# swapna267/flink

Measured on AMD Instinct MI355X. Metric: windowed-agg events/sec (whole node) at 1/2/4/8 GPU + % of HBM peak, higher is better.
Workload: dtype int64; 1 GPU; cfg2: Nexmark Q7-style TUMBLE(10 s) MAX(price) GROUP BY auction; plan=one-phase, keys_total=1000000, superbuckets=1024

## Files before the change

### flink_amd/csrc/fw_merge_impl.h

```cpp
#pragma once
#include <type_traits>

#include "fw_kernel_common.h"

namespace fw {
template <int NW, int E>
struct StateLds {
    static constexpr int NI = mg_idx_slots(NW, E);
    uint32_t idx[NI];
    int64_t key[E];
    int64_t slice[E];
    uint32_t flag[E];
    uint64_t acc[NW][E];
    uint16_t due[E];
    int32_t ndue;
    int32_t n;
    uint32_t overflow;
};

constexpr uint32_t IDX_DEAD = 0xFFFFFFFFu;

template <int W>
__device__ __forceinline__ void load_words(const uint64_t* p, uint64_t (&o)[W]) {
    if constexpr (W % 2 == 0) {
// ... 678 lines not shown
};
__device__ __forceinline__ CellGroup cell_group(uint32_t v, int f, int64_t CH) {
    const int lane = threadIdx.x & 63;
    const uint32_t cnt = cell_count(v);
    uint32_t inc = cnt;
#pragma unroll
    for (int d = 1; d < 64; d <<= 1) {
        const uint32_t t = (uint32_t)__shfl_up((int)inc, d, 64);
        if (lane >= d) inc += t;
    }
    CellGroup g;
    g.tot = (uint32_t)__shfl((int)inc, 63, 64);
    g.excl = inc - cnt;
    g.adj = (uint32_t)(cell_chunk(f) * CH + cell_start(v)) - g.excl;
    g.fmt = cell_fmt(v);
    return g;
}
constexpr int GF_PASS = 1;
constexpr int GF_COMPACT = 2;

struct PackDec {
    int64_t kbase, vbase, rbase;
    uint32_t ksh, rb, vb;
};
__device__ __forceinline__ PackDec pack_dec(const MergeArgs& a) {
    PackDec d;
    const uint32_t bits = __hip_atomic_load(&a.ctrl->pk_cur_bits, __ATOMIC_RELAXED, DEV_SCOPE);
    d.kbase = __hip_atomic_load(&a.ctrl->pk_cur_k, __ATOMIC_RELAXED, DEV_SCOPE);
    d.vbase = __hip_atomic_load(&a.ctrl->pk_cur_v, __ATOMIC_RELAXED, DEV_SCOPE);
    d.rbase = a.slot_base[0];
    d.ksh = 64u - (bits & 255u);
    d.rb = (bits >> 8) & 255u;
    d.vb = (bits >> 16) & 255u;
    return d;
}
template <int PW>
__device__ __forceinline__ void unpack_row(const PackDec& d, uint64_t w, int64_t interval, uint64_t (&row)[PW]) {
    static_assert(PW == 3, "PF_PACK rows carry one accumulator word");
    row[0] = (uint64_t)d.kbase + (w >> d.ksh);
    const uint32_t rank = (uint32_t)(w >> d.vb) & ((1u << d.rb) - 1u);
    row[1] = (uint64_t)(d.rbase + (int64_t)(rank * (uint32_t)interval));
    row[2] = (uint64_t)d.vbase + (w & ((1ull << d.vb) - 1ull));
}

template <int NW, int GU, int GF>
__device__ __forceinline__ uint32_t load_group_rows(const MergeArgs& a, int64_t pi, const CellGroup& g, uint32_t r0,
                                                    int sb, uint64_t (&row)[GU][2 + NW]) {
    constexpr int PW = 2 + NW;
    constexpr bool PS = (GF & GF_PASS) != 0, CR = (GF & GF_COMPACT) != 0;
    const int lane = threadIdx.x & 63;
    const uint64_t* seg = a.parts + (size_t)pi * a.cap_rows * PW;
#pragma unroll
    for (int u = 0; u < GU; u++) {
        const uint32_t x = min(r0 + (uint32_t)(u * 64 + lane), g.tot - 1);
        int lo = 0;
#pragma unroll
        for (int step = 32; step > 0; step >>= 1)
            if ((uint32_t)__shfl((int)g.excl, lo + step, 64) <= x) lo += step;
        const uint32_t rg = (uint32_t)__shfl((int)g.adj, lo, 64) + x;
        const uint32_t fmt = (uint32_t)__shfl((int)g.fmt, lo, 64);
        if (!CR || fmt == PF_WIDE) {
            load_words<PW>(seg + (size_t)rg * PW, row[u]);
        } else if (NW == 1 && fmt == PF_PACK) {
            const uint32_t within = rg & ((1u << a.ch_log2) - 1u);
            if constexpr (NW == 1) unpack_row(pack_dec(a), seg[(size_t)(rg - within) * PW + within], a.win.interval, row[u]);
        } else {
            const uint32_t within = rg & ((1u << a.ch_log2) - 1u);
            const uint64_t* p = seg + (size_t)(rg - within) * PW;
            const uint32_t rank = a.ranks[(size_t)pi * a.cap_rows + rg];
            row[u][1] = (uint64_t)(a.slot_base[pi] + (int64_t)(rank * (uint32_t)a.win.interval));
            if (fmt == PF_NARROW) {
                uint64_t t[1 + NW];
                load_words<1 + NW>(p + (size_t)within * (1 + NW), t);
                row[u][0] = t[0];
#pragma unroll
                for (int w = 0; w < NW; w++) row[u][2 + w] = t[1 + w];
            } else {
                row[u][0] = p[within];
#pragma unroll
                for (int w = 0; w < NW; w++) row[u][2 + w] = w == 0 ? 1ull : 0ull;
            }
        }
    }
    uint32_t live = 0;
#pragma unroll
    for (int u = 0; u < GU; u++) live |= (uint32_t)(r0 + (uint32_t)(u * 64 + lane) < g.tot) << u;
    if constexpr (PS)
#pragma unroll
        for (int u = 0; u < GU; u++) {
            uint32_t m;
            if ((live >> u) & 1u) live &= ~((uint32_t)(route_key(a.ks, (int64_t)row[u][0], 0, &m) != sb) << u);
        }
    return live;
}

static __device__ __noinline__ bool tz_fired_out_of_line(TzTable z, int64_t we, int64_t progress) {
    return tz_is_fired(z, we, progress);
}

static_assert(FW_MAX_PENDING * RUN_X <= 64, "one lane per (push, sub-run)");
struct RunSegs {
    uint32_t tot;
    uint32_t excl;
    uint32_t adj;
    uint32_t pf;
};
__device__ __forceinline__ RunSegs run_segs(const MergeArgs& a, int isb, int64_t pend) {
    const int lane = threadIdx.x & 63;
    const int p = lane / RUN_X, x = lane % RUN_X;
    uint32_t n = 0, fm = 0;
    if (p < pend) {
        n = min(a.run_fill[((size_t)p * RUN_X + x) * a.n_sb + isb], (uint32_t)a.sub_cap);
        fm = (uint32_t)a.slot_fmt[p];
    }
    uint32_t inc = n;
#pragma unroll
    for (int d = 1; d < 64; d <<= 1) {
        const uint32_t t = (uint32_t)__shfl_up((int)inc, d, 64);
        if (lane >= d) inc += t;
    }
    RunSegs g;
    g.tot = (uint32_t)__shfl((int)inc, 63, 64);
    g.excl = inc - n;
    g.adj = (uint32_t)(((size_t)isb * RUN_X + x) * (size_t)a.sub_cap) - g.excl;
    g.pf = (uint32_t)p | (fm << 4);
    return g;
}
template <int GU>
__device__ __forceinline__ uint32_t locate_run_rows(const RunSegs& g, uint32_t r0_, uint32_t (&ri)[GU], uint32_t (&pf)[GU]) {
    const int lane = threadIdx.x & 63;
    const uint32_t r0 = (uint32_t)__builtin_amdgcn_readfirstlane((int)r0_);
    const uint32_t tot = (uint32_t)__builtin_amdgcn_readfirstlane((int)g.tot);
    const uint32_t last = min(r0 + (uint32_t)(64 * GU), tot) - 1u;
    const uint32_t first = min(r0, tot - 1u);
    int cur = 0;
#pragma unroll
    for (int step = 32; step > 0; step >>= 1)
        if ((uint32_t)__builtin_amdgcn_readlane((int)g.excl, cur + step) <= first) cur += step;
    uint32_t x[GU], adj[GU];
    {
        const uint32_t a0 = (uint32_t)__builtin_amdgcn_readlane((int)g.adj, cur);
        const uint32_t p0 = (uint32_t)__builtin_amdgcn_readlane((int)g.pf, cur);
#pragma unroll
        for (int u = 0; u < GU; u++) {
            x[u] = min(r0 + (uint32_t)(u * 64 + lane), tot - 1u);
            adj[u] = a0;
            pf[u] = p0;
        }
    }
    while (cur < 63) {
        const uint32_t b = (uint32_t)__builtin_amdgcn_readlane((int)g.excl, cur + 1);
        if (b > last) break;
        cur++;
        const uint32_t an = (uint32_t)__builtin_amdgcn_readlane((int)g.adj, cur);
        const uint32_t pn = (uint32_t)__builtin_amdgcn_readlane((int)g.pf, cur);
#pragma unroll
        for (int u = 0; u < GU; u++) {
            adj[u] = x[u] >= b ? an : adj[u];
            pf[u] = x[u] >= b ? pn : pf[u];
        }
    }
    uint32_t live = 0;
#pragma unroll
    for (int u = 0; u < GU; u++) {
        ri[u] = adj[u] + x[u];
        live |= (uint32_t)(r0 + (uint32_t)(u * 64 + lane) < tot) << u;
    }
    return live;
}
template <int NW, int GU, int GF>
__device__ __forceinline__ uint32_t load_run_rows(const MergeArgs& a, const RunSegs& g, uint32_t r0_,
                                                  uint64_t (&row)[GU][2 + NW]) {
    constexpr int PW = 2 + NW;
    constexpr bool CR = (GF & GF_COMPACT) != 0;
    PackDec pk{};
    if constexpr (CR && NW == 1) pk = pack_dec(a);
    uint32_t rix[GU], pf[GU];
    const uint32_t live = locate_run_rows<GU>(g, r0_, rix, pf);
#pragma unroll
    for (int u = 0; u < GU; u++) {
        const uint32_t ri = rix[u];
        const uint32_t p = pf[u] & 15u, fmt = (pf[u] >> 4) & 3u;
        const uint64_t* base = a.runs + (size_t)p * a.run_rows * PW;
        if (!CR || fmt == PF_WIDE) {
            const uint64_t* q = base + (size_t)ri * PW;
#pragma unroll
            for (int w = 0; w < PW; w++) row[u][w] = q[w];
        } else if (NW == 1 && fmt == PF_PACK) {
            if constexpr (NW == 1) unpack_row(pk, base[ri], a.win.interval, row[u]);
        } else {
            const uint32_t rank = a.run_ranks[(size_t)p * a.run_rows + ri];
            row[u][1] = (uint64_t)(a.slot_base[p] + (int64_t)(rank * (uint32_t)a.win.interval));
            if (fmt == PF_NARROW) {
                uint64_t t[1 + NW];
                load_words<1 + NW>(base + (size_t)ri * (1 + NW), t);
                row[u][0] = t[0];
#pragma unroll
                for (int w = 0; w < NW; w++) row[u][2 + w] = t[1 + w];
            } else {
                row[u][0] = base[ri];
#pragma unroll
                for (int w = 0; w < NW; w++) row[u][2 + w] = w == 0 ? 1ull : 0ull;
            }
        }
    }
    return live;
}
template <int NW, int G, int GF, int D, typename F>
__device__ __forceinline__ void gather_runs(const MergeArgs& a, int sb, int64_t pend, F&& process) {
    constexpr int PW = 2 + NW;
    constexpr uint32_t STEP = (uint32_t)MG_BLOCK * G;
    const RunSegs g = run_segs(a, sb, pend);
    uint32_t r0 = (uint32_t)(threadIdx.x >> 6) * 64u * G;
    if (r0 >= g.tot) return;
    if constexpr (D > 1) {
        uint64_t buf[D][G][PW];
        uint32_t live[D];
        static_for<D - 1>([&](auto K) {
            constexpr int k = decltype(K)::value;
            live[k] = load_run_rows<NW, G, GF>(a, g, r0 + (uint32_t)k * STEP, buf[k]);
        });
        bool done = false;
        while (!done) {
            static_for<D>([&](auto K) {
                constexpr int k = decltype(K)::value;
                constexpr int kn = (k + D - 1) % D;
                if (done) return;
                live[kn] = load_run_rows<NW, G, GF>(a, g, r0 + (uint32_t)(D - 1) * STEP, buf[kn]);
                process(buf[k], live[k]);
                r0 += STEP;
                done = r0 >= g.tot;
            });
        }
    } else {
        for (; r0 < g.tot; r0 += STEP) {
            uint64_t row[G][PW];
            const uint32_t live = load_run_rows<NW, G, GF>(a, g, r0, row);
            process(row, live);
        }
    }
}
__device__ __forceinline__ uint32_t run_overflow(const MergeArgs& a, int sb, int64_t pend) {
    const int lane = threadIdx.x & 63;
    const bool o = lane < pend && a.run_ovf[(size_t)lane * a.n_sb + sb] != 0;
    return (uint32_t)__ballot(o);
}
__device__ __forceinline__ void run_release(const MergeArgs& a, int sb, int64_t pend) {
    const int t = threadIdx.x;
    if (t >= 64) return;
    const int p = t / RUN_X, x = t % RUN_X;
    if (p >= pend) return;
    a.run_fill[((size_t)p * RUN_X + x) * a.n_sb + sb] = 0u;
    if (x == 0) a.run_ovf[(size_t)p * a.n_sb + sb] = 0u;
}
template <int NW, int GU, int GF, typename F>
__device__ __forceinline__ void gather_cells_push(const MergeArgs& a, int sb, int64_t pi, F&& process) {
    constexpr int PW = 2 + NW;
    constexpr bool PS = (GF & GF_PASS) != 0;
    const int lane = threadIdx.x & 63, wv = threadIdx.x >> 6;
    const int ncell = (int)cell_pad(a.slot_nch[pi]);
    const int G = min(64, ncell / (MG_BLOCK / 64));
    const int ngroups = ncell / G;
    const int pl = PS ? a.ks.pass_log2 : 0;
    const int nis = a.n_sb >> pl;
    const uint32_t* cl = a.cells + (size_t)pi * nis * a.max_nch;
    for (int gi = wv; gi < ngroups; gi += MG_BLOCK / 64) {
        const int f = gi * G + lane;
        const uint32_t v = (lane >= G || cell_chunk(f) >= a.slot_nch[pi]) ? 0u : cl[((size_t)(f >> 4) * nis + (sb >> pl)) * CELL_LANES + (f & 15)];
        const CellGroup cg = cell_group(v, f, a.chunk_rows);
        for (uint32_t r0 = 0; r0 < cg.tot; r0 += 64 * GU) {
            uint64_t row[GU][PW];
            const uint32_t live = load_group_rows<NW, GU, GF>(a, pi, cg, r0, sb, row);
            process(row, live);
        }
    }
}

constexpr int GF_TAG = 4;
constexpr int MG_TAG_LOG2 = 13;
static_assert((1 << MG_TAG_LOG2) == MG_TAG_SLOTS, "tag_slot's shift");
constexpr uint32_t TG_DUE = 1u << 31;
#ifndef FW_TAG_G
#define FW_TAG_G 4
#endif
#ifndef FW_TAG_D
#define FW_TAG_D 1
#endif
struct TagLds {
    uint32_t tag[MG_TAG_SLOTS];
    uint64_t acc[MG_TAG_SLOTS];
    int64_t rk_end[MG_TAG_RANKS];
    uint32_t rk_flag[MG_TAG_RANKS];
    uint16_t due[MG_TAG_SLOTS];
    uint16_t live[MG_TAG_SLOTS];
    uint32_t ndue, nlive;
    uint32_t nfresh;
    uint32_t overflow;
};
struct TagEpoch {
    uint32_t bits;
    bool ok;
    int64_t kbase, vbase, rbase;
};
template <int NW, int E, bool TAG>
struct MergeLds {
    StateLds<NW, E> S;
};
template <int NW, int E>
struct MergeLds<NW, E, true> {
    union {
        StateLds<NW, E> S;
        TagLds T;
    };
};
__device__ __forceinline__ uint32_t tag_slot(uint32_t tg) { return (tg * 0x9E3779B1u) >> (32 - MG_TAG_LOG2); }

__device__ __forceinline__ TagEpoch tag_epoch(const MergeArgs& a, int64_t pend, bool flush) {
    TagEpoch ep;
    ep.bits = __hip_atomic_load(&a.ctrl->pk_cur_bits, __ATOMIC_RELAXED, DEV_SCOPE);
    ep.kbase = __hip_atomic_load(&a.ctrl->pk_cur_k, __ATOMIC_RELAXED, DEV_SCOPE);
    ep.vbase = __hip_atomic_load(&a.ctrl->pk_cur_v, __ATOMIC_RELAXED, DEV_SCOPE);
    ep.rbase = a.slot_base[0];
    bool pack = flush && (ep.bits & PK_OK) && (ep.bits & 255u) + ((ep.bits >> 8) & 255u) <= (uint32_t)MG_TAG_BITS;
    for (int p = 0; p < FW_MAX_PENDING; p++)
        if (p < pend) pack &= (uint32_t)a.slot_fmt[p] == PF_PACK;
    ep.ok = pack;
    return ep;
}

template <int G>
__device__ __forceinline__ uint32_t load_run_words(const MergeArgs& a, const RunSegs& g, uint32_t r0, uint64_t (&w)[G]) {
    uint32_t ri[G], pf[G];
    const uint32_t live = locate_run_rows<G>(g, r0, ri, pf);
#pragma unroll
    for (int u = 0; u < G; u++) w[u] = a.runs[(size_t)(pf[u] & 15u) * a.run_rows * 3 + ri[u]];
    return live;
}

template <uint32_t OPS, int G, int D>
__device__ __forceinline__ bool tag_superbucket(const MergeArgs& a, TagLds& T, int sb, int32_t n0, int64_t pend, int64_t W,
                                                int64_t w_old, bool do_fire, const TagEpoch& ep, Stamps& stm, int32_t* s_emit,
                                                int64_t* s_newmin) {
    constexpr int E = mg_entries(1, FW_WIN_TUMBLE);
    constexpr uint32_t MASK = MG_TAG_SLOTS - 1;
    constexpr int32_t OP = (int32_t)(OPS & 15u);
    const int tid = threadIdx.x;
    const uint32_t kb = ep.bits & 255u, rb = (ep.bits >> 8) & 255u, vb = (ep.bits >> 16) & 255u;
    const int64_t kbase = ep.kbase, vbase = ep.vbase, rbase = ep.rbase;
    const int64_t interval = a.win.interval;
    const uint64_t* st = a.state + (size_t)sb * a.cap_e * 4;
    uint64_t p[4] = {0, 0, 0, 0};
    if (tid < n0) load_words<4>(st + (size_t)tid * 4, p);
    auto claim = [&](uint32_t s, uint32_t tg) -> uint32_t {
        uint32_t was = 0;
        __hip_atomic_compare_exchange_strong(&T.tag[s], &was, tg, __ATOMIC_RELAXED, __ATOMIC_RELAXED, LDS_SCOPE);
        return was;
    };
    for (int i = tid; i < MG_TAG_SLOTS / 4; i += MG_BLOCK) ((uint4*)T.tag)[i] = make_uint4(0u, 0u, 0u, 0u);
    for (int i = tid; i < MG_TAG_SLOTS / 2; i += MG_BLOCK)
        ((ulonglong2*)T.acc)[i] = make_ulonglong2(word_identity(OP), word_identity(OP));
    if (tid < MG_TAG_RANKS) {
        const int64_t end = wadd(rbase, (int64_t)tid * interval);
        const uint32_t fl = is_fired(end, w_old) ? F_ACC : (F_ACC | F_TIMER);
        T.rk_end[tid] = end;
        T.rk_flag[tid] = fl | ((do_fire && (fl & F_TIMER) && is_fired(end, W)) ? TG_DUE : 0u);
    }
    if (tid == 0) {
        T.nfresh = 0;
        T.overflow = 0;
        T.ndue = 0;
        T.nlive = 0;
        *s_newmin = INT64_MAX;
    }
    __syncthreads();
    {
        const uint64_t span = (uint64_t)interval << rb;
        bool bad = false;
        for (int e = tid; e < n0; e += MG_BLOCK) {
            if (e != tid) load_words<4>(st + (size_t)e * 4, p);
            const uint64_t ko = p[0] - (uint64_t)kbase, d = p[1] - (uint64_t)rbase;
            const uint64_t r = udiv(d, a.win.slice_div);
            if (!(ko < (1ull << kb) && d < span && r * (uint64_t)interval == d && p[2] == (uint64_t)(F_ACC | F_TIMER) &&
                  !is_fired((int64_t)p[1], w_old))) {
                bad = true;
                continue;
            }
            const uint32_t tg = (((uint32_t)ko << rb) | (uint32_t)r) + 1u;
            uint32_t s = tag_slot(tg);
            while (claim(s, tg) != 0) s = (s + 1) & MASK;
            T.acc[s] = p[3];
        }
        if (__syncthreads_or(bad)) return false;
    }
    stm.mark(0);
    {
        const bool gst = (FW_ABL(a) & AB_GSTAMPS) && stm.on && tid == 0;
        uint64_t g0 = gst ? __builtin_amdgcn_s_memtime() : 0;
        const uint64_t gl0 = g0;
        auto gstamp = [&](int i, bool vm) {
            if (!gst) return;
            if (vm) asm volatile("s_waitcnt vmcnt(0)" ::: "memory");
            else asm volatile("s_waitcnt lgkmcnt(0)" ::: "memory");
            const uint64_t g1 = __builtin_amdgcn_s_memtime();
            stm.acc[i] += g1 - g0;
            g0 = g1;
        };
        const uint64_t vmask = (1ull << vb) - 1ull;
        uint32_t nfr = 0;
        auto fold_words = [&](uint64_t (&w)[G], uint32_t live) __attribute__((always_inline)) {
            gstamp(2, true);
            uint32_t tg[G], sl[G], was[G];
#pragma unroll
            for (int u = 0; u < G; u++) {
                tg[u] = (uint32_t)(w[u] >> vb) + 1u;
                sl[u] = tag_slot(tg[u]);
            }
#pragma unroll
            for (int u = 0; u < G; u++) was[u] = ((live >> u) & 1u) ? claim(sl[u], tg[u]) : tg[u];
            gstamp(4, false);
            uint32_t rest = 0;
#pragma unroll
            for (int u = 0; u < G; u++) {
                if (!((live >> u) & 1u)) continue;
                if (was[u] == 0 || was[u] == tg[u]) {
                    lds_fold(OP, &T.acc[sl[u]], (uint64_t)vbase + (w[u] & vmask));
                    nfr += was[u] == 0;
                } else {
                    rest |= 1u << u;
                }
            }
            while (rest) {
                const int um = __ffs(rest) - 1;
                rest &= rest - 1;
                uint64_t ww = 0;
                uint32_t t = 0, s = 0;
                static_for<G>([&](auto UU) {
                    constexpr int u = decltype(UU)::value;
                    if (u == um) {
                        ww = w[u];
                        t = tg[u];
                        s = sl[u];
                    }
                });
                for (int probes = 1;; probes++) {
                    s = (s + 1) & MASK;
                    const uint32_t o = claim(s, t);
                    if (o == 0 || o == t) {
                        lds_fold(OP, &T.acc[s], (uint64_t)vbase + (ww & vmask));
                        nfr += o == 0;
                        break;
                    }
                    if (probes >= MG_TAG_SLOTS) {
                        T.overflow = 1;
                        break;
                    }
                }
            }
            gstamp(7, false);
        };
        constexpr uint32_t STEP = (uint32_t)MG_BLOCK * G;
        const RunSegs g = run_segs(a, sb, pend);
        uint32_t r0 = (uint32_t)(tid >> 6) * 64u * G;
        if (r0 < g.tot) {
            if constexpr (D > 1) {
                uint64_t buf[D][G];
                uint32_t live[D];
                static_for<D - 1>([&](auto K) {
                    constexpr int k = decltype(K)::value;
                    live[k] = load_run_words<G>(a, g, r0 + (uint32_t)k * STEP, buf[k]);
                });
                bool done = false;
                while (!done) {
                    static_for<D>([&](auto K) {
                        constexpr int k = decltype(K)::value;
                        constexpr int kn = (k + D - 1) % D;
                        if (done) return;
                        live[kn] = load_run_words<G>(a, g, r0 + (uint32_t)(D - 1) * STEP, buf[kn]);
                        fold_words(buf[k], live[k]);
                        r0 += STEP;
                        done = r0 >= g.tot;
                    });
                }
            } else {
                for (; r0 < g.tot; r0 += STEP) {
                    uint64_t w[G];
                    const uint32_t live = load_run_words<G>(a, g, r0, w);
                    fold_words(w, live);
                }
            }
            nfr = wred_sum_u32(nfr);
            if ((tid & 63) == 0 && nfr) __hip_atomic_fetch_add(&T.nfresh, nfr, __ATOMIC_RELAXED, LDS_SCOPE);
        }
        if (gst) stm.acc[13] += __builtin_amdgcn_s_memtime() - gl0;
    }
    __syncthreads();
    stm.mark(1);
    run_release(a, sb, pend);
    const uint32_t n_ent = (uint32_t)n0 + T.nfresh;
    const uint32_t rmask = (1u << rb) - 1u;
    {
        constexpr int PER = MG_TAG_SLOTS / MG_BLOCK;
        uint32_t tgs[PER];
#pragma unroll
        for (int j = 0; j < PER; j++) tgs[j] = T.tag[j * MG_BLOCK + tid];
        uint32_t isdue = 0, islive = 0, nd = 0, nl = 0;
        uint64_t bd[PER], bl[PER];
#pragma unroll
        for (int j = 0; j < PER; j++) {
            const uint32_t fl = tgs[j] ? T.rk_flag[(tgs[j] - 1u) & rmask] : 0u;
            isdue |= (uint32_t)((fl & TG_DUE) != 0) << j;
            islive |= (uint32_t)(fl != 0 && !(fl & TG_DUE)) << j;
            bd[j] = __ballot((isdue >> j) & 1u);
            bl[j] = __ballot((islive >> j) & 1u);
            nd += (uint32_t)__popcll(bd[j]);
            nl += (uint32_t)__popcll(bl[j]);
        }
        uint32_t d0 = 0, l0 = 0;
        if ((tid & 63) == 0) {
            if (nd) d0 = __hip_atomic_fetch_add(&T.ndue, nd, __ATOMIC_RELAXED, LDS_SCOPE);
            if (nl) l0 = __hip_atomic_fetch_add(&T.nlive, nl, __ATOMIC_RELAXED, LDS_SCOPE);
        }
        d0 = uni32(d0);
        l0 = uni32(l0);
#pragma unroll
        for (int j = 0; j < PER; j++) {
            const uint32_t rd = __builtin_amdgcn_mbcnt_hi((uint32_t)(bd[j] >> 32), __builtin_amdgcn_mbcnt_lo((uint32_t)bd[j], 0u));
            const uint32_t rl = __builtin_amdgcn_mbcnt_hi((uint32_t)(bl[j] >> 32), __builtin_amdgcn_mbcnt_lo((uint32_t)bl[j], 0u));
            if ((isdue >> j) & 1u) T.due[d0 + rd] = (uint16_t)(j * MG_BLOCK + tid);
            if ((islive >> j) & 1u) T.live[l0 + rl] = (uint16_t)(j * MG_BLOCK + tid);
            d0 += (uint32_t)__popcll(bd[j]);
            l0 += (uint32_t)__popcll(bl[j]);
        }
    }
    __syncthreads();
    stm.mark(6);
    const uint32_t ndue = T.ndue, nlive = min(T.nlive, (uint32_t)a.cap_e);
    for (uint32_t q = tid; q < ndue; q += MG_BLOCK) {
        const uint32_t sl = T.due[q], x = T.tag[sl] - 1u;
        uint64_t acc[1] = {T.acc[sl]};
        if (a.ad.count_star_word < 0 || acc[0] != 0)
            emit_row<1, false>(a, sb, s_emit, wadd(kbase, (int64_t)(x >> rb)), T.rk_end[x & rmask], acc);
    }
    stm.mark(5);
    {
        uint64_t* so = a.state + (size_t)sb * a.cap_e * 4;
        int64_t lnm = INT64_MAX;
        for (uint32_t q = tid; q < nlive; q += MG_BLOCK) {
            const uint32_t sl = T.live[q], x = T.tag[sl] - 1u, fl = T.rk_flag[x & rmask];
            const int64_t end = T.rk_end[x & rmask];
            st16(so + (size_t)q * 4, (uint64_t)wadd(kbase, (int64_t)(x >> rb)), (uint64_t)end);
            st16(so + (size_t)q * 4 + 2, (uint64_t)(fl & (F_ACC | F_TIMER)), T.acc[sl]);
            if (fl & F_TIMER) lnm = min(lnm, end);
        }
        lnm = wred_min_i64(lnm);
        if ((tid & 63) == 0 && lnm != INT64_MAX) __hip_atomic_fetch_min(s_newmin, lnm, __ATOMIC_RELAXED, LDS_SCOPE);
    }
    __syncthreads();
    if (tid == 0) {
        a.state_count[sb] = (int32_t)nlive;
        a.sb_min_timer[sb] = *s_newmin;
        a.sb_out[sb] = (int32_t)min((int64_t)*s_emit, a.slab_cap);
        if (ndue) a.sb_fired[sb] += ndue;
        __hip_atomic_fetch_add(&a.ctrl->state_moved, (uint64_t)(n0 + (int32_t)nlive), __ATOMIC_RELAXED, DEV_SCOPE);
        __hip_atomic_fetch_max(&a.ctrl->peak_entries, (uint64_t)n_ent, __ATOMIC_RELAXED, DEV_SCOPE);
        if (T.overflow || n_ent > (uint32_t)E) __hip_atomic_fetch_or(&a.ctrl->error, ERR_STATE, __ATOMIC_RELAXED, DEV_SCOPE);
    }
    __syncthreads();
    stm.mark(3);
    return true;
}

template <int NW, int E, bool Q, int KIND, uint32_t OPS, int GF>
__global__ __launch_bounds__(MG_BLOCK, 4) void k_merge_fire(MergeArgs a) {
    constexpr bool PS = (GF & GF_PASS) != 0;
    constexpr bool TAG = (GF & GF_TAG) != 0;
    static_assert(!TAG || (NW == 1 && KIND == FW_WIN_TUMBLE && !Q && !PS && OPS != OPS_ANY && E == mg_entries(1, FW_WIN_TUMBLE)),
                  "the tag path serves the one-word SQL TUMBLE layouts");
    constexpr int PW = 2 + NW;
    constexpr int PWE = 3 + NW;
    const int64_t CH = a.chunk_rows;
    constexpr int GU = mg_rows_in_flight(NW);
    __shared__ MergeLds<NW, E, TAG> lds;
    StateLds<NW, E>& S = lds.S;
    __shared__ int32_t s_work;
    __shared__ int32_t s_nlive;
    __shared__ int64_t s_newmin;
    __shared__ uint32_t s_fired;
    __shared__ int32_t s_emit;

    const int tid = threadIdx.x;
    kt_start(a.kt);
    Ctrl* c = a.ctrl;
    const int64_t W = merge_watermark(a);
    const MergeDecision d = merge_decide<KIND>(a, W);
    const int64_t pend = d.pend, ntreq = d.ntreq, nlf = d.nlf, w_old = d.cur;
    const bool do_flush = d.do_flush, do_fire = d.do_fire;

    Stamps stm;
    stm.init((FW_ABL(a) & AB_STAMPS) != 0);
    TagEpoch tep{};
    uint32_t n_by_path[2] = {0, 0};
    if constexpr (TAG) tep = tag_epoch(a, pend, do_flush && ntreq == 0 && !(FW_ABL(a) & ~(AB_STAMPS | AB_GSTAMPS)));
    const bool xq = a.n_sb % 8 == 0 && gridDim.x % 8 == 0;
    const int nq = xq ? a.n_sb / 8 : a.n_sb;
    uint32_t* const wq = &a.tickets->work[xq ? blockIdx.x % 8 : 0][0];
    const int qbase = xq ? (int)(blockIdx.x % 8) * nq : 0;
    __shared__ int32_t s_tk;
    if (tid == 0) s_tk = (int32_t)__hip_atomic_fetch_add(wq, 1u, __ATOMIC_RELAXED, DEV_SCOPE);
    if (!do_flush && ntreq == 0) {
        bool due = false;
        for (int i = tid; i < nq; i += MG_BLOCK) due |= do_fire && win_fired(a.win, a.sb_min_timer[qbase + i], W);
        if (!__syncthreads_or(due)) {
            if (a.reset_out)
                for (int i = tid; i < nq; i += MG_BLOCK) a.sb_out[qbase + i] = 0;
            s_tk = nq;
        }
    }
    __syncthreads();
    for (int tk = s_tk; tk < nq; tk = s_tk) {
    const int sb = qbase + tk;
    const int32_t n0 = a.state_count[sb];
    uint32_t ovf_w = 0;
    if constexpr (TAG)
        if (tep.ok && (tid & 63) < pend) ovf_w = a.run_ovf[(size_t)(tid & 63) * a.n_sb + sb];
    __syncthreads();
    if (tid == 0) {
        s_tk = (int32_t)__hip_atomic_fetch_add(wq, 1u, __ATOMIC_RELAXED, DEV_SCOPE);
        s_work = (ntreq > 0) || do_flush || (do_fire && win_fired(a.win, a.sb_min_timer[sb], W));
        s_fired = 0;
        s_emit = a.reset_out ? 0 : a.sb_out[sb];
        if (!s_work && a.reset_out) a.sb_out[sb] = 0;
    }
    __syncthreads();
    if (!s_work) continue;
    if constexpr (TAG) {
        const bool tagp = tep.ok && __ballot(ovf_w != 0) == 0;
        const bool served = tagp && tag_superbucket<OPS, FW_TAG_G, FW_TAG_D>(a, lds.T, sb, n0, pend, W, w_old, do_fire, tep, stm,
                                                                              &s_emit, &s_newmin);
        n_by_path[served]++;
        if (served) continue;
    }
    const bool gather = do_flush && !(FW_ABL(a) & AB_M_NO_GATHER);
    auto cell_at = [&](int64_t pi, int f) -> uint32_t {
        if (cell_chunk(f) >= a.slot_nch[pi]) return 0u;
        const int pl = PS ? a.ks.pass_log2 : 0;
        const int nis = a.n_sb >> pl;
        const uint32_t* cl = a.cells + (size_t)pi * nis * a.max_nch;
        return cl[((size_t)(f >> 4) * nis + (sb >> pl)) * CELL_LANES + (f & 15)];
    };
    const int lane = tid & 63, wv = tid >> 6;
    auto gather_group = [](int ncell) { return min(64, ncell / (MG_BLOCK / 64)); };
    uint32_t v_first = 0;
    if (gather && !a.runs && lane < gather_group((int)cell_pad(a.slot_nch[0])))
        v_first = cell_at(0, wv * gather_group((int)cell_pad(a.slot_nch[0])) + lane);
    for (int i = tid; i < StateLds<NW, E>::NI; i += MG_BLOCK) S.idx[i] = 0;
    if (tid == 0) {
        S.n = (FW_ABL(a) & AB_M_NO_LOAD) ? 0 : n0;
        S.overflow = 0;
        S.ndue = 0;
    }
    __syncthreads();
    const uint64_t* st = a.state + (size_t)sb * a.cap_e * PWE;
    if (!(FW_ABL(a) & AB_M_NO_LOAD)) for (int e = tid; e < n0; e += MG_BLOCK) {
        uint64_t p[PWE];
        load_words<PWE>(st + (size_t)e * PWE, p);
        const int64_t k = (int64_t)p[0], s = (int64_t)p[1];
        S.key[e] = k;
        S.slice[e] = s;
        S.flag[e] = (uint32_t)p[2];
#pragma unroll
        for (int w = 0; w < NW; w++) S.acc[w][e] = p[3 + w];
        uint32_t h = index_hash(k, s) & (StateLds<NW, E>::NI - 1);
        for (;;) {
            uint32_t expect = 0;
            if (__hip_atomic_compare_exchange_strong(&S.idx[h], &expect, 2u + (uint32_t)e, __ATOMIC_RELAXED,
                                                     __ATOMIC_RELAXED, LDS_SCOPE))
                break;
            h = (h + 1) & (StateLds<NW, E>::NI - 1);
        }
    }
    __syncthreads();
    stm.mark(0);
    for (int64_t r = tid; r < ntreq; r += MG_BLOCK) {
        if (a.treq[3 * r + 2] != sb) continue;
        const int e = find_or_insert<NW, E, OPS>(S, a.treq[3 * r], a.treq[3 * r + 1], a.wd);
        if (e >= 0) atomicOr(&S.flag[e], F_TIMER);
    }
    const bool gst = (FW_ABL(a) & AB_GSTAMPS) && stm.on && tid == 0;
    constexpr bool PIPE = NW >= 2 && NW <= 4 && (KIND == FW_WIN_TUMBLE || KIND == FW_WIN_CUMULATE);
    if (gather && a.runs) {
        const bool utc = a.win.tz.n == 0;
        auto flags_of = [&](int64_t sl) -> uint32_t {
            const bool fired = a.local || (utc ? is_fired(sl, w_old) : tz_fired_out_of_line(a.win.tz, sl, w_old));
            return fired ? F_ACC : (F_ACC | F_TIMER);
        };
        auto fold_rows = [&](auto& row, uint32_t live) __attribute__((always_inline)) {
            constexpr int GX = std::extent<std::remove_reference_t<decltype(row)>>::value;
            if (FW_ABL(a) & AB_M_NO_HASH) {
                uint64_t x = 0;
#pragma unroll
                for (int u = 0; u < GX; u++) x ^= row[u][0] ^ row[u][1] ^ row[u][PW - 1];
                asm volatile("" ::"v"(x));
                return;
            }
            if constexpr (KIND == KIND_DSWIN) {
                static_for<GX>([&](auto UU) {
                    constexpr int u = decltype(UU)::value;
                    if ((live >> u) & 1u)
                        ds_add_to_windows<NW, E>(a, S, (int64_t)row[u][0], (int64_t)row[u][1], &row[u][2], w_old, false);
                });
            } else {
                uint64_t g0 = gst ? __builtin_amdgcn_s_memtime() : 0;
                auto gstamp = [&](int i) {
                    if (!gst) return;
                    asm volatile("s_waitcnt lgkmcnt(0)" ::: "memory");
                    const uint64_t g1 = __builtin_amdgcn_s_memtime();
                    stm.acc[i] += g1 - g0;
                    g0 = g1;
                };
                int ge[GX];
                auto probe_fold = [&](uint32_t want) __attribute__((always_inline)) -> uint32_t {
                    {
                        int64_t gk[GX], gs[GX];
#pragma unroll
                        for (int u = 0; u < GX; u++) {
                            gk[u] = (int64_t)row[u][0];
                            gs[u] = (int64_t)row[u][1];
                        }
                        probe_batch<NW, E, GX>(S, gk, gs, ge, GX, want);
                    }
                    uint32_t rest = 0;
                    static_for<GX>([&](auto UU) {
                        constexpr int u = decltype(UU)::value;
                        if (!((want >> u) & 1u)) return;
                        const int e = ge[u];
                        if (e < 0) {
                            rest |= 1u << u;
                            return;
                        }
                        if (FW_ABL(a) & AB_M_NO_FOLDOP) return;
#pragma unroll
                        for (int w = 0; w < NW; w++)
                            if (word_on<OPS>(a.wd, w)) lds_fold(word_op<OPS>(a.wd, w), &S.acc[w][e], row[u][2 + w]);
                        atomicOr(&S.flag[e], flags_of((int64_t)row[u][1]));
                    });
                    return rest;
                };
                uint32_t miss = probe_fold(live);
                gstamp(4);
                const bool gcount = (FW_ABL(a) & AB_GSTAMPS) && stm.on && (tid >> 6) == 0;
                if (gcount) {
                    uint32_t lv = 0, fr = 0, ud = 0;
#pragma unroll
                    for (int u = 0; u < GX; u++)
                        if ((live >> u) & 1u) {
                            lv++;
                            fr += ge[u] == -1;
                            ud += ge[u] == -2;
                        }
                    lv = wave_sum_u32(lv);
                    fr = wave_sum_u32(fr);
                    ud = wave_sum_u32(ud);
                    if (tid == 0) {
                        stm.acc[8] += lv;
                        stm.acc[9] += fr;
                        stm.acc[10] += ud;
                    }
                }
                miss = insert_fresh<NW, E, GX, OPS>(S, a.wd, row, miss, ge, flags_of);
                if (gcount) {
                    const uint32_t sl = wave_sum_u32((uint32_t)__popc(miss));
                    if (tid == 0) stm.acc[11] += sl;
                }
                gstamp(14);
                while (miss) {
                    const int um = __ffs(miss) - 1;
                    miss &= miss - 1;
                    if (gst) stm.acc[12]++;
                    uint64_t r[PW];
                    static_for<GX>([&](auto UU) {
                        constexpr int u = decltype(UU)::value;
                        if (u == um) {
#pragma unroll
                            for (int w = 0; w < PW; w++) r[w] = row[u][w];
                        }
                    });
                    const uint32_t fl = flags_of((int64_t)r[1]);
                    bool ins = false;
                    const int e = find_or_insert<NW, E, OPS>(S, (int64_t)r[0], (int64_t)r[1], a.wd, &r[2], fl, &ins);
                    if (e < 0 || ins || (FW_ABL(a) & AB_M_NO_FOLDOP)) continue;
#pragma unroll
                    for (int w = 0; w < NW; w++)
                        if (word_on<OPS>(a.wd, w)) lds_fold(word_op<OPS>(a.wd, w), &S.acc[w][e], r[2 + w]);
                    atomicOr(&S.flag[e], fl);
                }
                gstamp(7);
            }
        };
        constexpr bool RP = NW <= 4 && (KIND == FW_WIN_TUMBLE || KIND == FW_WIN_CUMULATE);
        constexpr bool ONE_BLOCK = NW == 1 && KIND == FW_WIN_TUMBLE;
        constexpr int GR = !RP ? GU : ONE_BLOCK ? 4 : GU / 2 > 0 ? GU / 2 : 1;
        constexpr int GD = !RP ? 1 : ONE_BLOCK ? 1 : 2;
        const uint64_t gl0 = gst ? __builtin_amdgcn_s_memtime() : 0;
        gather_runs<NW, GR, GF, GD>(a, sb, pend, fold_rows);
        if (gst) stm.acc[13] += __builtin_amdgcn_s_memtime() - gl0;
        uint32_t ovf = run_overflow(a, sb, pend);
        while (ovf) {
            const int pi = __ffs(ovf) - 1;
            ovf &= ovf - 1;
            gather_cells_push<NW, GU, GF>(a, sb, pi, fold_rows);
        }
    } else if (PIPE && gather) {
        constexpr int GP = NW == 1 ? GU : GU / 2 > 0 ? GU / 2 : 1;
        const bool utc = a.win.tz.n == 0;
        auto flags_of = [&](int64_t sl) -> uint32_t {
            const bool fired = a.local || (utc ? is_fired(sl, w_old) : tz_fired_out_of_line(a.win.tz, sl, w_old));
            return fired ? F_ACC : (F_ACC | F_TIMER);
        };
        auto ngroups_of = [&](int64_t p) {
            const int nc = (int)cell_pad(a.slot_nch[p]);
            return nc / gather_group(nc);
        };
        auto norm = [&](int64_t& p, int& q) {
            while (p < pend && q >= ngroups_of(p)) {
                p++;
                q = wv;
            }
        };
        auto fpos = [&](int64_t p, int q) { return q * gather_group((int)cell_pad(a.slot_nch[p])) + lane; };
        auto cword = [&](int64_t p, int q) -> uint32_t {
            return lane < gather_group((int)cell_pad(a.slot_nch[p])) ? cell_at(p, fpos(p, q)) : 0u;
        };
        CellGroup cg;
        cg.tot = cg.excl = cg.adj = cg.fmt = 0;
        int64_t cp = 0;
        uint32_t r0 = 0;
        int64_t np = 0;
        int nq = wv;
        norm(np, nq);
        uint32_t vn = np < pend ? ((np == 0 && nq == wv) ? v_first : cword(np, nq)) : 0u;
        auto next_block = [&]() -> bool {
            r0 += 64 * GP;
            while (r0 >= cg.tot) {
                if (np >= pend) return false;
                const uint32_t vc = vn;
                const int f = fpos(np, nq);
                cp = np;
                nq += MG_BLOCK / 64;
                norm(np, nq);
                vn = np < pend ? cword(np, nq) : 0u;
                cg = cell_group(vc, f, CH);
                r0 = 0;
            }
            return true;
        };
        auto process = [&](auto& row, uint32_t live) {
            constexpr int GX = std::extent<std::remove_reference_t<decltype(row)>>::value;
            if (FW_ABL(a) & AB_M_NO_HASH) {
                uint64_t x = 0;
#pragma unroll
                for (int u = 0; u < GX; u++) x ^= row[u][0] ^ row[u][1] ^ row[u][PW - 1];
                asm volatile("" ::"v"(x));
                return;
            }
            int ge[GX];
            {
                int64_t gk[GX], gs[GX];
#pragma unroll
                for (int u = 0; u < GX; u++) {
                    gk[u] = (int64_t)row[u][0];
                    gs[u] = (int64_t)row[u][1];
                }
                probe_batch<NW, E, GX>(S, gk, gs, ge);
            }
            uint32_t miss = 0;
            static_for<GX>([&](auto UU) {
                constexpr int u = decltype(UU)::value;
                if (!((live >> u) & 1u)) return;
                const int e = ge[u];
                if (e < 0) {
                    miss |= 1u << u;
                    return;
                }
                if (FW_ABL(a) & AB_M_NO_FOLDOP) return;
#pragma unroll
                for (int w = 0; w < NW; w++)
                    if (word_on<OPS>(a.wd, w)) lds_fold(word_op<OPS>(a.wd, w), &S.acc[w][e], row[u][2 + w]);
                atomicOr(&S.flag[e], flags_of((int64_t)row[u][1]));
            });
            while (miss) {
                const int um = __ffs(miss) - 1;
                miss &= miss - 1;
                uint64_t r[PW];
                static_for<GX>([&](auto UU) {
                    constexpr int u = decltype(UU)::value;
                    if (u == um) {
#pragma unroll
                        for (int w = 0; w < PW; w++) r[w] = row[u][w];
                    }
                });
                const uint32_t fl = flags_of((int64_t)r[1]);
                bool ins = false;
                const int e = find_or_insert<NW, E, OPS>(S, (int64_t)r[0], (int64_t)r[1], a.wd, &r[2], fl, &ins);
                if (e < 0 || ins || (FW_ABL(a) & AB_M_NO_FOLDOP)) continue;
#pragma unroll
                for (int w = 0; w < NW; w++)
                    if (word_on<OPS>(a.wd, w)) lds_fold(word_op<OPS>(a.wd, w), &S.acc[w][e], r[2 + w]);
                atomicOr(&S.flag[e], fl);
            }
        };
        uint64_t ra[GP][PW], rb[GP][PW];
        uint32_t la = 0, lb = 0;
        bool ha = next_block();
        if (ha) la = load_group_rows<NW, GP, GF>(a, cp, cg, r0, sb, ra);
        while (ha) {
            const bool hb = next_block();
            if (hb) lb = load_group_rows<NW, GP, GF>(a, cp, cg, r0, sb, rb);
            process(ra, la);
            if (!hb) break;
            ha = next_block();
            if (ha) la = load_group_rows<NW, GP, GF>(a, cp, cg, r0, sb, ra);
            process(rb, lb);
        }
    } else if (gather) {
        for (int64_t pi = 0; pi < pend; pi++) {
            const int ncell = (int)cell_pad(a.slot_nch[pi]);
            const int G = gather_group(ncell);
            const int ngroups = ncell / G;
            for (int g = wv; g < ngroups; g += MG_BLOCK / 64) {
                const int f = g * G + lane;
                uint64_t gc0 = gst ? __builtin_amdgcn_s_memtime() : 0;
                const uint32_t v = lane >= G ? 0u : g == wv ? v_first : cell_at(pi, f);
                    if (g == wv) {
                        v_first = 0;
                        if (pi + 1 < pend) {
                            const int G1 = gather_group((int)cell_pad(a.slot_nch[pi + 1]));
                            if (lane < G1) v_first = cell_at(pi + 1, wv * G1 + lane);
                        }
                    }
                if (gst) {
                    asm volatile("s_waitcnt vmcnt(0)" ::: "memory");
                    const uint64_t g1 = __builtin_amdgcn_s_memtime();
                    stm.acc[13] += g1 - gc0;
                    gc0 = g1;
// ... 399 lines not shown
```

Before: 49.04 billion events/s.

## Batch-prefetch superbucket headers into LDS and overlap next ticket fetch in tag path

Adds a per-block LDS header cache that loads run fill counts, overflow bits, state counts and sb_out for up to 128 superbuckets at once, coalesced across threads. The tag path then reads these from LDS instead of issuing small scattered global loads per superbucket. It also fetches the next work ticket early, right after the fold phase, so that atomic's latency overlaps with the emit phase. The trade-offs are extra LDS use, a refill when tickets jump outside the cached window, and a new sub_cap < 65536 requirement for the tag path because fills are stored as 16-bit values.

```diff
diff --git a/flink_amd/csrc/fw_merge_impl.h b/flink_amd/csrc/fw_merge_impl.h
--- a/flink_amd/csrc/fw_merge_impl.h
+++ b/flink_amd/csrc/fw_merge_impl.h
@@ -1004,6 +1004,27 @@
     bool ok;
     int64_t kbase, vbase, rbase;
 };
+constexpr int MG_HDR_FILLS = FW_MAX_PENDING * RUN_X;
+template <int HB>
+struct TagHdr {
+    int32_t sb_out[HB];
+    uint16_t n0[HB];
+    uint16_t ovf[HB];
+    uint16_t fill[HB][MG_HDR_FILLS + 2];
+};
+constexpr int MG_LDS_BYTES = 160 * 1024;
+constexpr int MG_LDS_SCALARS = 64;
+constexpr int MG_TAG_HB = 128;
+static_assert(sizeof(TagLds) + sizeof(TagHdr<MG_TAG_HB>) + MG_LDS_SCALARS <= MG_LDS_BYTES &&
+                  sizeof(TagLds) + sizeof(TagHdr<2 * MG_TAG_HB>) + MG_LDS_SCALARS > MG_LDS_BYTES,
+              "MG_TAG_HB: the largest power of two that fits the LDS");
+static_assert(MG_BLOCK % MG_TAG_HB == 0 && MG_BLOCK / MG_TAG_HB >= 3 && MG_HDR_FILLS % (MG_BLOCK / MG_TAG_HB) == 0,
+              "tag_hdr_fill's deal of the header's arrays to the threads");
+using TagHeaders = TagHdr<MG_TAG_HB>;
+struct TagPart {
+    TagLds T;
+    TagHeaders H;
+};
 template <int NW, int E, bool TAG>
 struct MergeLds {
     StateLds<NW, E> S;
@@ -1012,9 +1033,64 @@
 struct MergeLds<NW, E, true> {
     union {
         StateLds<NW, E> S;
-        TagLds T;
+        TagPart tp;
     };
 };
+static_assert(sizeof(TagPart) <= sizeof(StateLds<1, mg_entries(1, FW_WIN_TUMBLE)>) &&
+                  sizeof(MergeLds<1, mg_entries(1, FW_WIN_TUMBLE), true>) + MG_LDS_SCALARS <= MG_LDS_BYTES,
+              "the tag table and the headers fit the entry table's LDS");
+static __device__ __noinline__ void tag_hdr_fill(const uint32_t* run_fill, const uint32_t* run_ovf, const int32_t* state_count,
+                                                 const int32_t* sb_out, int n_sb, uint32_t sub_cap, TagHeaders* H, int sb0,
+                                                 int cnt, int pend) {
+    constexpr int HB = MG_TAG_HB, ROWS = MG_BLOCK / HB, PER = MG_HDR_FILLS / ROWS;
+    const int col = threadIdx.x % HB, row = threadIdx.x / HB;
+    if (col >= cnt) return;
+    const int sb = sb0 + col;
+    const int nfill = pend * RUN_X;
+    uint32_t f[PER];
+#pragma unroll
+    for (int k = 0; k < PER; k++) {
+        const int j = row + k * ROWS;
+        f[k] = j < nfill ? run_fill[(size_t)j * n_sb + sb] : 0u;
+    }
+    uint32_t v = 0;
+    if (row == 0) {
+#pragma unroll
+        for (int p = 0; p < FW_MAX_PENDING; p++)
+            if (p < pend) v |= (uint32_t)(run_ovf[(size_t)p * n_sb + sb] != 0) << p;
+    } else if (row == 1) {
+        v = (uint32_t)state_count[sb];
+    } else if (row == 2) {
+        v = (uint32_t)sb_out[sb];
+    }
+#pragma unroll
+    for (int k = 0; k < PER; k++) H->fill[col][row + k * ROWS] = (uint16_t)min(f[k], sub_cap);
+    if (row == 0) H->ovf[col] = (uint16_t)v;
+    else if (row == 1) H->n0[col] = (uint16_t)v;
+    else if (row == 2) H->sb_out[col] = (int32_t)v;
+}
+__device__ __forceinline__ RunSegs run_segs_hdr(const MergeArgs& a, const TagHeaders& H, int hi, int isb, int64_t pend) {
+    int lane = threadIdx.x & 63;
+    asm volatile("" : "+v"(lane));
+    const int p = lane / RUN_X, x = lane % RUN_X;
+    uint32_t n = 0, fm = 0;
+    if (p < pend) {
+        n = H.fill[hi][lane];
+        fm = PF_PACK;
+    }
+    uint32_t inc = n;
+#pragma unroll
+    for (int d = 1; d < 64; d <<= 1) {
+        const uint32_t t = (uint32_t)__shfl_up((int)inc, d, 64);
+        if (lane >= d) inc += t;
+    }
+    RunSegs g;
+    g.tot = (uint32_t)__shfl((int)inc, 63, 64);
+    g.excl = inc - n;
+    g.adj = (uint32_t)(((size_t)isb * RUN_X + x) * (size_t)a.sub_cap) - g.excl;
+    g.pf = (uint32_t)p | (fm << 4);
+    return g;
+}
 __device__ __forceinline__ uint32_t tag_slot(uint32_t tg) { return (tg * 0x9E3779B1u) >> (32 - MG_TAG_LOG2); }
 
 __device__ __forceinline__ TagEpoch tag_epoch(const MergeArgs& a, int64_t pend, bool flush) {
@@ -1023,7 +1099,8 @@
     ep.kbase = __hip_atomic_load(&a.ctrl->pk_cur_k, __ATOMIC_RELAXED, DEV_SCOPE);
     ep.vbase = __hip_atomic_load(&a.ctrl->pk_cur_v, __ATOMIC_RELAXED, DEV_SCOPE);
     ep.rbase = a.slot_base[0];
-    bool pack = flush && (ep.bits & PK_OK) && (ep.bits & 255u) + ((ep.bits >> 8) & 255u) <= (uint32_t)MG_TAG_BITS;
+    bool pack = flush && (ep.bits & PK_OK) && (ep.bits & 255u) + ((ep.bits >> 8) & 255u) <= (uint32_t)MG_TAG_BITS &&
+                a.sub_cap < 65536;
     for (int p = 0; p < FW_MAX_PENDING; p++)
         if (p < pend) pack &= (uint32_t)a.slot_fmt[p] == PF_PACK;
     ep.ok = pack;
@@ -1040,9 +1117,9 @@
 }
 
 template <uint32_t OPS, int G, int D>
-__device__ __forceinline__ bool tag_superbucket(const MergeArgs& a, TagLds& T, int sb, int32_t n0, int64_t pend, int64_t W,
-                                                int64_t w_old, bool do_fire, const TagEpoch& ep, Stamps& stm, int32_t* s_emit,
-                                                int64_t* s_newmin) {
+__device__ __forceinline__ bool tag_superbucket(const MergeArgs& a, TagLds& T, const TagHeaders& H, int hi, int sb, int32_t n0,
+                                                int64_t pend, int64_t W, int64_t w_old, bool do_fire, const TagEpoch& ep,
+                                                Stamps& stm, int32_t* s_emit, int64_t* s_newmin, uint32_t* wq, int32_t* s_tk) {
     constexpr int E = mg_entries(1, FW_WIN_TUMBLE);
     constexpr uint32_t MASK = MG_TAG_SLOTS - 1;
     constexpr int32_t OP = (int32_t)(OPS & 15u);
@@ -1052,7 +1129,9 @@
     const int64_t interval = a.win.interval;
     const uint64_t* st = a.state + (size_t)sb * a.cap_e * 4;
     uint64_t p[4] = {0, 0, 0, 0};
-    if (tid < n0) load_words<4>(st + (size_t)tid * 4, p);
+    int t0 = tid;
+    asm volatile("" : "+v"(t0));
+    if (t0 < n0) load_words<4>(st + (size_t)t0 * 4, p);
     auto claim = [&](uint32_t s, uint32_t tg) -> uint32_t {
         uint32_t was = 0;
         __hip_atomic_compare_exchange_strong(&T.tag[s], &was, tg, __ATOMIC_RELAXED, __ATOMIC_RELAXED, LDS_SCOPE);
@@ -1073,6 +1152,7 @@
         T.ndue = 0;
         T.nlive = 0;
         *s_newmin = INT64_MAX;
+        *s_emit = a.reset_out ? 0 : H.sb_out[hi];
     }
     __syncthreads();
     {
@@ -1161,7 +1241,7 @@
             gstamp(7, false);
         };
         constexpr uint32_t STEP = (uint32_t)MG_BLOCK * G;
-        const RunSegs g = run_segs(a, sb, pend);
+        const RunSegs g = run_segs_hdr(a, H, hi, sb, pend);
         uint32_t r0 = (uint32_t)(tid >> 6) * 64u * G;
         if (r0 < g.tot) {
             if constexpr (D > 1) {
@@ -1197,6 +1277,8 @@
     }
     __syncthreads();
     stm.mark(1);
+    int32_t tk_next = 0;
+    if (tid == 0) tk_next = (int32_t)__hip_atomic_fetch_add(wq, 1u, __ATOMIC_RELAXED, DEV_SCOPE);
     run_release(a, sb, pend);
     const uint32_t n_ent = (uint32_t)n0 + T.nfresh;
     const uint32_t rmask = (1u << rb) - 1u;
@@ -1266,6 +1348,7 @@
         __hip_atomic_fetch_add(&a.ctrl->state_moved, (uint64_t)(n0 + (int32_t)nlive), __ATOMIC_RELAXED, DEV_SCOPE);
         __hip_atomic_fetch_max(&a.ctrl->peak_entries, (uint64_t)n_ent, __ATOMIC_RELAXED, DEV_SCOPE);
         if (T.overflow || n_ent > (uint32_t)E) __hip_atomic_fetch_or(&a.ctrl->error, ERR_STATE, __ATOMIC_RELAXED, DEV_SCOPE);
+        *s_tk = tk_next;
     }
     __syncthreads();
     stm.mark(3);
@@ -1308,7 +1391,16 @@
     uint32_t* const wq = &a.tickets->work[xq ? blockIdx.x % 8 : 0][0];
     const int qbase = xq ? (int)(blockIdx.x % 8) * nq : 0;
     __shared__ int32_t s_tk;
-    if (tid == 0) s_tk = (int32_t)__hip_atomic_fetch_add(wq, 1u, __ATOMIC_RELAXED, DEV_SCOPE);
+    int hbase = 0;
+    if constexpr (TAG) {
+        int32_t tk0 = 0;
+        if (tid == 0) tk0 = (int32_t)__hip_atomic_fetch_add(wq, 1u, __ATOMIC_RELAXED, DEV_SCOPE);
+        if (tep.ok)
+            tag_hdr_fill(a.run_fill, a.run_ovf, a.state_count, a.sb_out, a.n_sb, (uint32_t)a.sub_cap, &lds.tp.H, qbase, min(MG_TAG_HB, nq), (int)pend);
+        if (tid == 0) s_tk = tk0;
+    } else {
+        if (tid == 0) s_tk = (int32_t)__hip_atomic_fetch_add(wq, 1u, __ATOMIC_RELAXED, DEV_SCOPE);
+    }
     if (!do_flush && ntreq == 0) {
         bool due = false;
         for (int i = tid; i < nq; i += MG_BLOCK) due |= do_fire && win_fired(a.win, a.sb_min_timer[qbase + i], W);
@@ -1321,10 +1413,25 @@
     __syncthreads();
     for (int tk = s_tk; tk < nq; tk = s_tk) {
     const int sb = qbase + tk;
+    if constexpr (TAG) {
+        if (tep.ok) {
+            const int tku = __builtin_amdgcn_readfirstlane(tk);
+            if ((uint32_t)(tku - hbase) >= (uint32_t)MG_TAG_HB) {
+                hbase = tku & ~(MG_TAG_HB - 1);
+                tag_hdr_fill(a.run_fill, a.run_ovf, a.state_count, a.sb_out, a.n_sb, (uint32_t)a.sub_cap, &lds.tp.H, qbase + hbase,
+                             min(MG_TAG_HB, nq - hbase), (int)pend);
+                __syncthreads();
+            }
+            const int hi = tku - hbase;
+            const bool served = lds.tp.H.ovf[hi] == 0 &&
+                                tag_superbucket<OPS, FW_TAG_G, FW_TAG_D>(a, lds.tp.T, lds.tp.H, hi, sb, (int32_t)lds.tp.H.n0[hi], pend, W,
+                                                                         w_old, do_fire, tep, stm, &s_emit, &s_newmin, wq, &s_tk);
+            n_by_path[served]++;
+            if (served) continue;
+            hbase = -MG_TAG_HB;
+        }
+    }
     const int32_t n0 = a.state_count[sb];
-    uint32_t ovf_w = 0;
-    if constexpr (TAG)
-        if (tep.ok && (tid & 63) < pend) ovf_w = a.run_ovf[(size_t)(tid & 63) * a.n_sb + sb];
     __syncthreads();
     if (tid == 0) {
         s_tk = (int32_t)__hip_atomic_fetch_add(wq, 1u, __ATOMIC_RELAXED, DEV_SCOPE);
@@ -1335,13 +1442,8 @@
     }
     __syncthreads();
     if (!s_work) continue;
-    if constexpr (TAG) {
-        const bool tagp = tep.ok && __ballot(ovf_w != 0) == 0;
-        const bool served = tagp && tag_superbucket<OPS, FW_TAG_G, FW_TAG_D>(a, lds.T, sb, n0, pend, W, w_old, do_fire, tep, stm,
-                                                                              &s_emit, &s_newmin);
-        n_by_path[served]++;
-        if (served) continue;
-    }
+    if constexpr (TAG)
+        if (!tep.ok) n_by_path[0]++;
     const bool gather = do_flush && !(FW_ABL(a) & AB_M_NO_GATHER);
     auto cell_at = [&](int64_t pi, int f) -> uint32_t {
         if (cell_chunk(f) >= a.slot_nch[pi]) return 0u;
```

New measurement: 49.96 billion events/s (median of 6 runs). About the same (+1.9%).
